# NIRVANALAN/CVPR23-E3DGE

Hardware: AMD Instinct MI355X
Metric: rendered_rays_per_sec_64x64x24 (higher is better)
Workload: dtype f32 (operands split f16 hi+lo, 3 f16 MFMA products, fp32 accumulate)

## Files before the change

cvpr23-e3dge_amd/_lib.py:

```python
import ctypes
import operator
import os
import threading
import weakref

_HERE = os.path.dirname(os.path.abspath(__file__))
LIB_PATH = os.environ.get("E3DGE_LIB_PATH") or os.path.join(_HERE, "lib", "libe3dge_hip.so")
ABI_VERSION = 17
PREC_F32, PREC_F16X3, PREC_F16X3_V1, PREC_F16X3_G2 = 0, 1, 2, 3
AMAX_FLOATS = 64 * 32
MC_MAX_TRIS = 16

_c_float_p = ctypes.c_void_p
_i32, _i64, _f32, _vp = ctypes.c_int, ctypes.c_int64, ctypes.c_float, ctypes.c_void_p


class _Args(ctypes.Structure):

    def __init__(self, *values, **fields):
        if values:
            fields = dict(zip((f[0] for f in self._fields_), values), **fields)
        seen = None
        for name, value in fields.items():
            kind = value.__class__
# ... 80 lines not shown
class Dec2Rgb(_Args):
    _fields_ = [(n, _vp) for n in ("weight", "style", "bias", "wm", "out")] + [("scale", _f32), ("ci", _i32)]


class Dec2Plan(_Args):
    _fields_ = [("batch", _i32), ("n_up", _i32), ("in_res", _i32), ("in_ch", _i32),
                ("features", _vp), ("skip_in", _vp), ("mod_table", _vp), ("latent", _vp),
                ("n_mod", _i32), ("mod_rows", _i32), ("mod_co", _i32), ("n_latent", _i32), ("style_dim", _i32), ("reserved0", _i32),
                ("conv1", Dec2Conv), ("rgb1", Dec2Rgb),
                ("up", Dec2Conv * DEC2_MAX_UP), ("conv", Dec2Conv * DEC2_MAX_UP), ("rgb", Dec2Rgb * DEC2_MAX_UP),
                ("act", _vp * (2 * DEC2_MAX_UP + 2)), ("amax", _vp), ("meta", _vp),
                ("fir_blur", _vp), ("fir_up", _vp), ("negative_slope", _f32), ("act_scale", _f32),
                ("kernel_ms", ctypes.POINTER(ctypes.c_float)), ("n_kernel_ms", _i32), ("reserved1", _i32),
                ("fir_blur_1d", _f32 * 4), ("fir_blur_separable", _i32), ("save_for_backward", _i32)]


class Dec2BwdConv(_Args):
    _fields_ = [(n, _vp) for n in ("wpre_t", "wcol", "wimg_t")]


class Dec2BwdPlan(_Args):
    _fields_ = [("d_img", _vp), ("d_features", _vp), ("conv1", Dec2BwdConv), ("up", Dec2BwdConv * DEC2_MAX_UP),
                ("conv", Dec2BwdConv * DEC2_MAX_UP), ("gact", _vp * (2 * DEC2_MAX_UP + 2)), ("pbuf", _vp),
                ("drgb", _vp * DEC2_MAX_UP), ("amax", _vp), ("meta", _vp), ("bounds", _vp),
                ("kernel_ms", ctypes.POINTER(ctypes.c_float)), ("n_kernel_ms", _i32), ("reserved", _i32),
                ("d_latent", _vp), ("ds_part", _vp), ("ds_part_floats", _i64)]


class WsLinear(_Args):
    _fields_ = [(n, _vp) for n in ("wimg", "x", "amax_in", "bias", "colw", "m", "r1", "r2", "y", "amax_out")] + [("n_rows", _i64)] + [
        (n, _i32) for n in ("ld_x", "off_x", "ld_m", "off_m", "ld_r1", "off_r1", "ld_r2", "off_r2", "ld_y", "off_y", "pre_relu", "post")] + [
        ("slope", _f32), ("w_fuse", _f32), ("xmul", _vp), ("amax_xmul", _vp), ("ld_xmul", _i32), ("off_xmul", _i32), ("x_scale", _f32),
        ("reserved", _i32)]


class Wgrad(_Args):
    _fields_ = [(n, _vp) for n in ("a", "amax_a", "b", "amax_b", "c", "ws")] + [("ws_floats", _i64), ("n_rows", _i64)] + [
        (n, _i32) for n in ("lda", "off_a", "m", "ldb", "off_b", "n", "ldc", "relu_b")] + [(n, _vp) for n in ("xcol", "colsum", "ccol")] + [
        (n, _i32) for n in ("ld_xcol", "ld_ccol", "b_gap_at", "b_gap")]


MESH_MAX_FACES_PER_PIXEL = 8


class MeshRenderArgs(_Args):
    _fields_ = [(n, _vp) for n in ("verts", "faces", "normals", "colors")] + [("n_verts", _i64), ("n_faces", _i64), ("camera", _f32 * 12),
               ("tan_half_fov", _f32), ("znear", _f32), ("zfar", _f32)] + [
        (n, _f32 * 3) for n in ("light_location", "ambient_color", "diffuse_color", "specular_color", "background_color")] + [
        ("blur_radius", _f32), ("sigma", _f32), ("gamma", _f32), ("image_size", _i32), ("faces_per_pixel", _i32)] + [
        (n, _vp) for n in ("image", "zbuf", "pix_to_face", "status", "ws")] + [("ws_bytes", _i64), ("bin_capacity", _i64)]


NOISE_PROJECT_FACES_PER_PIXEL, NOISE_PROJECT_MAX_MAPS = 17, 4


class NoiseProjectArgs(_Args):
    _fields_ = [(n, _vp) for n in ("verts", "faces", "vert_noise", "prev")] + [("n_verts", _i64), ("n_faces", _i64), ("camera", _f32 * 12)] + [
        (n, _f32) for n in ("tan_half_fov", "znear", "zfar", "blur_radius", "sigma", "gamma")] + [("image_size", _i32), ("n_maps", _i32)] + [
        (n, _vp) for n in ("out", "valid", "status", "ws")] + [("ws_bytes", _i64), ("bin_capacity", _i64)]


LPIPS_LAYERS = 5


class LpipsArgs(_Args):
    _fields_ = [(n, _vp) for n in ("packed", "x", "y")] + [(n, _i32) for n in ("batch", "height", "width", "reserved")] + [
# ... 197 lines not shown
    "e3dge_idnet_embed": (_i32, [ctypes.POINTER(IdnetArgs), _vp]),
    "e3dge_id_loss": (_i32, [ctypes.POINTER(IdLossArgs), _vp]),
    "e3dge_idnet_conv_tiles": (_i32, [_i32] * 5),
    "e3dge_idnet_conv": (_i32, [_vp] * 8 + [_i32] * 7 + [_vp]),
    "e3dge_idnet_packed_t_floats": (_i64, []),
    "e3dge_idnet_pack_weights_t": (_i32, [_vp, _vp, _vp]),
    "e3dge_idnet_saved_bytes": (_i64, [_i32]),
    "e3dge_idnet_embed_save": (_i32, [ctypes.POINTER(IdnetSaveArgs), _vp]),
    "e3dge_idnet_bwd_ws_bytes": (_i64, [_i32, _i32, _i32]),
    "e3dge_idnet_backward": (_i32, [ctypes.POINTER(IdnetBwdArgs), _vp]),
    "e3dge_idnet_conv_bwd": (_i32, [_vp] * 9 + [_i32] * 7 + [_vp]),
    "e3dge_idnet_prep_bwd": (_i32, [_vp, _vp, _i32, _i32, _i32, _vp]),
    "e3dge_hitprob_points": (_i32, [_vp] * 8 + [_i32, _i64, _i32, _i32, _vp]),
    "e3dge_hitprob_composite": (_i32, [_vp] * 6 + [_f32, _i32, _i32, _i64, _i32, _i32, _vp]),
    "e3dge_align_volume": (_i32, [_vp, _vp, _vp, _vp, _vp, _vp, _i32, _i32, _i32, _i32, _i32, _vp]),
    "e3dge_marching_cubes_ws_bytes": (_i64, [_i32, _i32, _i32]),
    "e3dge_marching_cubes_count": (_i32, [_vp, _vp, _i64, _vp, _i32, _i32, _i32, _i64, _i64, _i64, _vp]),
    "e3dge_marching_cubes_emit": (_i32, [_vp, _vp, _i64, _i64, _vp, _i64, _vp, _i32, _i32, _i32, _i64, _i64, _i64, _i32, _vp]),
    "e3dge_marching_cubes_tables": (_i32, [_vp, _vp]),
    "e3dge_depth_mesh": (_i32, [_vp, _vp, _vp, _i32, _i32, _vp]),
    "e3dge_vertex_normals_ws_bytes": (_i64, [_i64]),
    "e3dge_vertex_normals": (_i32, [_vp, _vp, _vp, _i64, _i64, _vp, _i64, _vp]),
    "e3dge_mesh_render_ws_bytes": (_i64, [_i64, _i64, _i32, _i64]),
    "e3dge_mesh_render": (_i32, [ctypes.POINTER(MeshRenderArgs), _vp]),
    "e3dge_mesh_subdivide": (_i32, [_vp, _vp, _vp, _vp, _vp, _vp, _i64, _i64, _i64, _vp]),
    "e3dge_noise_project_ws_bytes": (_i64, [_i64, _i64, _i32, _i64]),
    "e3dge_noise_project": (_i32, [ctypes.POINTER(NoiseProjectArgs), _vp]),
    "e3dge_selftest_mfma": (_i32, [_vp, _vp, _vp, _i32, _vp]),
    "e3dge_selftest_mfma16": (_i32, [_vp, _vp, _vp, _i32, _vp]),
    "e3dge_selftest_mfma16x16": (_i32, [_vp, _vp, _vp, _i32, _vp]),
    "e3dge_ws_image_bytes": (_i64, [_i32]),
    "e3dge_ws_pack": (_i32, [_vp, _vp, _i32, _vp]),
    "e3dge_ws_linear": (_i32, [ctypes.POINTER(WsLinear), _vp]),
    "e3dge_ws_rowdot2": (_i32, [_vp, _i32, _i32, _vp, _vp, _vp, _vp, _vp, _i32, _i32, _i64, _vp]),
    "e3dge_selftest_sin": (_i32, [_vp, _vp, _i32, _vp]),
    "e3dge_selftest_sin_poly": (_i32, [_vp, _vp, _i32, _vp]),
    "e3dge_avgpool_fwd": (_i32, [_vp, _vp, _i64, _i32, _i32, _i32, _vp]),
    "e3dge_avgpool_bwd": (_i32, [_vp, _vp, _i64, _i32, _i32, _i32, _vp]),
    "e3dge_sqerr_bwd": (_i32, [_vp, _vp, _vp, _i64, _vp, _vp]),
    "e3dge_shape_loss_partial_floats": (_i64, [ctypes.POINTER(ShapeLossArgs)]),
    "e3dge_shape_loss_fwd": (_i32, [ctypes.POINTER(ShapeLossArgs), _vp]),
    "e3dge_shape_loss_bwd": (_i32, [ctypes.POINTER(ShapeLossArgs), _vp]),
    "e3dge_disc_packed_floats": (_i64, [_i32] * 3),
    "e3dge_disc_pack_weights": (_i32, [_vp, _vp, _vp]),
    "e3dge_disc_ws_bytes": (_i64, [_i32] * 7),
    "e3dge_disc_saved_bytes": (_i64, [_i32] * 4),
    "e3dge_disc_forward": (_i32, [ctypes.POINTER(DiscArgs), _vp]),
    "e3dge_disc_backward": (_i32, [ctypes.POINTER(DiscBwdArgs), _vp]),
    "e3dge_disc_conv": (_i32, [_vp] * 6 + [_i32] * 9 + [_f32, _vp]),
    "e3dge_disc_conv_dgrad": (_i32, [_vp] * 5 + [_f32, _f32, _vp] + [_i32] * 7 + [_f32, _vp]),
    "e3dge_disc_stddev": (_i32, [_vp, _vp, _vp, _i32, _i32, _i32, _vp]),
    "e3dge_hgf_packed_floats": (_i64, [_i32, _i32]),
    "e3dge_hgf_pack_weights": (_i32, [_vp, _vp, _i32, _vp, _i32, _i32, _vp]),
    "e3dge_hgf_ws_bytes": (_i64, [_i32] * 5),
    "e3dge_hgf_forward": (_i32, [ctypes.POINTER(HgfArgs), _vp]),
    "e3dge_hgf_front": (_i32, [_vp] * 4 + [_i32] * 5 + [_vp, _i64, _vp]),
    "e3dge_hgf_conv": (_i32, [_vp] * 8 + [_i32] * 12 + [_vp]),
    "e3dge_hgf_norm": (_i32, [_vp] * 4 + [_i32] * 7 + [_vp]),
    "e3dge_hgf_pool": (_i32, [_vp, _vp, _i64, _i32, _i32, _vp]),
    "e3dge_hgf_up_add": (_i32, [_vp, _vp, _vp, _i64, _i32, _i32, _vp]),
    "e3dge_hgf_saved_bytes": (_i64, [_i32] * 5),
    "e3dge_hgf_forward_saving": (_i32, [ctypes.POINTER(HgfArgs), _vp, _i64, _vp]),
    "e3dge_hgf_front_saving": (_i32, [_vp] * 4 + [_i32] * 5 + [_vp, _i64, _vp, _i64, _vp]),
    "e3dge_hgf_packed_t_floats": (_i64, [_i32, _i32]),
    "e3dge_hgf_pack_weights_t": (_i32, [_vp, _vp, _i32, _vp, _i32, _i32, _vp]),
    "e3dge_hgf_bwd_ws_bytes": (_i64, [_i32] * 5),
# ... 266 lines not shown
```

cvpr23-e3dge_amd/build.py:

```python
import hashlib
import os
import shutil
import subprocess
import sys

HERE = os.path.dirname(os.path.abspath(__file__))
CSRC = os.path.join(HERE, "csrc")
LIBDIR = os.path.join(HERE, "lib")
LIBNAME = "libe3dge_hip.so"
SOURCES = ["stream_ops.hip", "upfirdn2d.hip", "siren.hip", "siren_bwd.hip", "resblock.hip", "modconv.hip", "decoder2.hip", "local_query.hip", "metrics.hip", "align_volume.hip", "hitprob.hip", "siren_ws.hip", "wgrad.hip",
           "marching_cubes.hip", "mesh_render.hip", "lpips.hip", "idnet.hip", "losses.hip", "disc.hip", "hgfilter.hip", "aligner.hip"]
ARCH = "gfx950"
FLAGS = ["-O3", "-std=c++17", "-fPIC", f"--offload-arch={ARCH}", "-ffp-contract=on", "-fno-slp-vectorize",
         "-Wno-unused-result"]


def lib_path():
    return os.path.join(LIBDIR, LIBNAME)


def _hipcc():
    for cand in (os.environ.get("HIPCC"), shutil.which("hipcc"), "/opt/rocm/bin/hipcc"):
        if cand and os.path.exists(cand):
            return cand
    raise RuntimeError("hipcc not found (set HIPCC=...)")


def _digest():
    h = hashlib.sha256()
    for name in sorted(os.listdir(CSRC)) + ["../../include/e3dge_hip.h"]:
        with open(os.path.join(CSRC, name), "rb") as f:
            h.update(name.encode() + b"\0" + f.read())
    h.update(" ".join(FLAGS).encode())
    return h.hexdigest()


def _compile(pairs, flags, verbose, jobs):
    hipcc = _hipcc()
    todo, running = list(pairs), []
    while todo or running:
        while todo and len(running) < jobs:
            src, obj = todo.pop(0)
            cmd = [hipcc, *flags, "-c", os.path.join(CSRC, src), "-o", obj]
# ... 63 lines not shown
```

cvpr23-e3dge_amd/local_query.py:

```python
import os

import torch
from torch import nn

from . import _lib


def fuse_autograd_backend():
    v = os.environ.get("E3DGE_FUSE_AUTOGRAD", "hip")
    if v not in ("hip", "torch"):
        raise RuntimeError(f"E3DGE_FUSE_AUTOGRAD must be 'hip' or 'torch', got {v!r}")
    return v


def native_fuse_backend():
    v = os.environ.get("E3DGE_FUSE", "hip")
    if v not in ("hip", "torch"):
        raise RuntimeError(f"E3DGE_FUSE must be 'hip' or 'torch', got {v!r}")
    return v


def query_feature_map(pts, calibs, fmap=None, out=None, col_off=0, mask_out=None, mask_off=0, want_proj=False):
    _lib.require_gpu(pts, "pts")
    _lib.require_gpu(calibs, "calibs")
# ... 178 lines not shown
        if fc0.out_features != 256 or self.encode_enc.fc_1.out_features != 256 or fc0.in_features not in (512, 513):
            return False
        if enc_in.shape[-1] != fc0.in_features or self.encode_enc.shortcut is None:
            return False
        return all(p.device == enc_in.device and p.dtype == torch.float32 for p in _lib.params_of(self))

    def _fusefn_ok(self, enc_in, dec_feat, w):
        if enc_in.numel() == 0 or (torch.is_tensor(w) and (w.requires_grad or w.numel() != 1)):
            return False
        b_off = enc_in.shape[-1] - 256
        tail = enc_in[..., b_off:]
        return (torch.is_tensor(dec_feat) and dec_feat.shape == tail.shape and dec_feat.data_ptr() == tail.data_ptr()
                and dec_feat.stride() == tail.stride())

    def _wants_grad(self, enc_in):
        return torch.is_grad_enabled() and (enc_in.requires_grad or any(p.requires_grad for p in _lib.params_of(self)))

    def _param_list(self):
        e = self.encode_enc
        return [e.fc_0.weight, e.fc_0.bias, e.fc_1.weight, e.fc_1.bias, e.shortcut.weight,
                self.scale[0].weight, self.scale[0].bias, self.scale[2].weight, self.scale[2].bias,
                self.shift[0].weight, self.shift[0].bias, self.shift[2].weight, self.shift[2].bias]

    def invalidate(self):
        _lib.invalidate(self)

    def _images(self, device):
        return _lib.cached(self, 'images', _lib.params_of(self), self._build_images, (str(device),))

    def _build_images(self):
        enc, n_in = self.encode_enc, self.encode_enc.fc_0.in_features
        has_col = n_in == 513
        b_off = 257 if has_col else 256
        img = _ws_image
        f0, sc = enc.fc_0.weight, enc.shortcut.weight
        return dict(b_off=b_off, has_col=has_col,
                    f0a=img(f0[:, :256]), f0b=img(f0[:, b_off:]), f1=img(enc.fc_1.weight), sa=img(sc[:, :256]), sb=img(sc[:, b_off:]),
                    sc1=img(self.scale[0].weight), sc2=img(self.scale[2].weight), sh1=img(self.shift[0].weight), sh2=img(self.shift[2].weight),
                    f0col=f0[:, 256].detach().contiguous() if has_col else None, scol=sc[:, 256].detach().contiguous() if has_col else None,
                    b0=enc.fc_0.bias.detach().contiguous(), b1=enc.fc_1.bias.detach().contiguous(),
                    bsc1=self.scale[0].bias.detach().contiguous(), bsc2=self.scale[2].bias.detach().contiguous(),
                    bsh1=self.shift[0].bias.detach().contiguous(), bsh2=self.shift[2].bias.detach().contiguous(),
                    slope=float(self.scale[1].negative_slope))

    def _images_t(self, device):
        I = self._images(device)
        if 'sc2_t' not in I:
            enc, b_off = self.encode_enc, I['b_off']
            img_t = lambda w: _ws_image(w.t())
            f0, sc = enc.fc_0.weight, enc.shortcut.weight
            I.update(sc2_t=img_t(self.scale[2].weight), sh2_t=img_t(self.shift[2].weight), sc1_t=img_t(self.scale[0].weight),
                     sh1_t=img_t(self.shift[0].weight), f1_t=img_t(enc.fc_1.weight), sa_t=img_t(sc[:, :256]), sb_t=img_t(sc[:, b_off:]),
                     f0a_t=img_t(f0[:, :256]), f0b_t=img_t(f0[:, b_off:]))
        return I

    def _fuse_bwd_native(self, g, x, net, s1, t1, scale, am_x, w, b_off, slope, need_x, ld_g=256, mask_col=True):
        N = g.shape[0]
        dev = g.device
        ld = x.shape[1]
        I = self._images_t(dev)
        f32 = dict(device=dev, dtype=torch.float32)
        dz1, dz2, de, dnet = (torch.empty((N, 256), **f32) for _ in range(4))
        dx = torch.empty((N, ld), **f32) if need_x else None
        am = torch.zeros((5, _lib.AMAX_FLOATS), **f32)

        def lin(wimg, xin, am_in, y, ld_x=256, ld_y=256, off_y=0, post=0, sl=0.0, r1=None, r1_ld=256, r1_off=0, r2=None, r2_ld=256, r2_off=0,
                xmul=None, amax_out=None, x_scale=1.0):
            a = _lib.WsLinear()
            a.wimg, a.x, a.amax_in, a.y, a.amax_out = wimg, xin, am_in, y, amax_out
            a.r1, a.r2 = r1, r2
            a.n_rows = N
            a.ld_x, a.off_x, a.ld_y, a.off_y = ld_x, 0, ld_y, off_y
            a.ld_r1, a.off_r1, a.ld_r2, a.off_r2, a.ld_m, a.off_m = r1_ld, r1_off, r2_ld, r2_off, 1, 0
            a.post, a.slope, a.w_fuse, a.x_scale = post, sl, w, x_scale
            if xmul is not None:
                a.xmul, a.amax_xmul, a.ld_xmul, a.off_xmul = xmul, am_x, ld, b_off
# ... 2 lines not shown
            _lib.launch("e3dge_amax", am[0], g, g.numel())
        else:
            _lib.launch("e3dge_amax_rows", am[0], g, N, 256, ld_g)
        lin(I['sc2_t'], g, am[0], dz1, ld_x=ld_g, post=3, sl=slope, r1=s1, xmul=x, x_scale=w, amax_out=am[1])
        lin(I['sh2_t'], g, am[0], dz2, ld_x=ld_g, post=3, sl=slope, r1=t1, x_scale=w, amax_out=am[2])
        lin(I['sc1_t'], dz1, am[1], de)
        lin(I['sh1_t'], dz2, am[2], de, r1=de, amax_out=am[3])
        lin(I['f1_t'], de, am[3], dnet, post=3, sl=0.0, r1=net, amax_out=am[4])
        if need_x:
            lin(I['sa_t'], de, am[3], dx, ld_y=ld, off_y=0)
            lin(I['f0a_t'], dnet, am[4], dx, ld_y=ld, off_y=0, post=3, sl=0.0, r1=x, r1_ld=ld, r1_off=0, r2=dx, r2_ld=ld, r2_off=0)
            lin(I['sb_t'], de, am[3], dx, ld_y=ld, off_y=b_off, post=4, r1=g, r1_ld=ld_g, r2=scale)
            lin(I['f0b_t'], dnet, am[4], dx, ld_y=ld, off_y=b_off, post=3, sl=0.0, r1=x, r1_ld=ld, r1_off=b_off, r2=dx, r2_ld=ld, r2_off=b_off)
        if need_x and I['has_col'] and not mask_col:
            dx[:, 256].zero_()
        if need_x and I['has_col'] and mask_col:
            _lib.launch("e3dge_ws_rowdot2", dx, ld, 256, de, I['scol'], dnet, I['f0col'], x, ld, 256, N)
        return dz1, dz2, de, dnet, dx, am

    def _fuse_native(self, enc_in, w, out, out_off, keep=None):
        lead = enc_in.shape[:-1]
        x = _lib.dense(enc_in.reshape(-1, enc_in.shape[-1]))
        N, ld = x.shape
        dev = x.device
        I = self._images(dev)
        if out is None:
            out = torch.empty(lead + (256,), device=dev, dtype=torch.float32)
            out_off = 0
        o2 = out.reshape(-1, out.shape[-1])
        if o2.data_ptr() != out.data_ptr() or not o2.is_contiguous():
            raise RuntimeError("Fuse_sft_MLP.fuse: `out` must be a contiguous (..., ld) buffer")
        if N == 0:
            return out[..., out_off:out_off + 256]
        A, Bf, C = (torch.empty((N, 256), device=dev, dtype=torch.float32) for _ in range(3))
        if keep is not None:
            NET, E, S1, T1 = (torch.empty((N, 256), device=dev, dtype=torch.float32) for _ in range(4))
        else:
            NET, E, S1, T1 = Bf, Bf, A, A
        am = torch.zeros((5, _lib.AMAX_FLOATS), device=dev, dtype=torch.float32)
        b_off = I['b_off']

        def lin(wimg, xin, ld_x, off_x, amax_in, y, ld_y=256, off_y=0, bias=None, col=None, r1=None, r1_ld=256, r1_off=0, r2=None,
                pre_relu=False, post=0, amax_out=None):
            a = _lib.WsLinear()
            a.wimg, a.x, a.amax_in, a.bias = wimg, xin, amax_in, bias
            a.colw, a.m = (col, x) if col is not None else (None, None)
            a.r1, a.r2, a.y, a.amax_out = r1, r2, y, amax_out
            a.n_rows = N
            a.ld_x, a.off_x, a.ld_m, a.off_m = ld_x, off_x, ld, 256
            a.ld_r1, a.off_r1, a.ld_r2, a.off_r2, a.ld_y, a.off_y = r1_ld, r1_off, 256, 0, ld_y, off_y
            a.pre_relu, a.post, a.slope, a.w_fuse = int(pre_relu), post, I['slope'], w
            _lib.launch("e3dge_ws_linear", a)
        _lib.launch("e3dge_amax", am[0], x, x.numel())
        lin(I['f0a'], x, ld, 0, am[0], A, pre_relu=True)
        lin(I['f0b'], x, ld, b_off, am[0], NET, bias=I['b0'], col=I['f0col'], r1=A, pre_relu=True, amax_out=am[1])
        lin(I['f1'], NET, 256, 0, am[1], A, bias=I['b1'], pre_relu=True)
        lin(I['sa'], x, ld, 0, am[0], C)
        lin(I['sb'], x, ld, b_off, am[0], E, col=I['scol'], r1=C, r2=A, amax_out=am[2])
        lin(I['sc1'], E, 256, 0, am[2], S1, bias=I['bsc1'], post=1, amax_out=am[3])
        lin(I['sc2'], S1, 256, 0, am[3], C, bias=I['bsc2'])
        lin(I['sh1'], E, 256, 0, am[2], T1, bias=I['bsh1'], post=1, amax_out=am[4])
        lin(I['sh2'], T1, 256, 0, am[4], o2, ld_y=o2.shape[-1], off_y=out_off, bias=I['bsh2'], r1=x, r1_ld=ld, r1_off=b_off, r2=C, post=2)
        if keep is not None:
            keep.update(x=x, net=NET, e=E, s1=S1, t1=T1, scale=C, b_off=b_off, slope=I['slope'], am_x=am[0], am=am)
        return out[..., out_off:out_off + 256]


class _FuseFn(torch.autograd.Function):

    @staticmethod
    def forward(ctx, mod, enc_in, w, pe_pts, n_freqs, mask_col_const, *params):
        keep = {}
        with torch.no_grad():
            if pe_pts is None:
                out = mod._fuse_native(enc_in.detach(), w, None, 0, keep=keep)
            else:
                width = 3 * (2 * n_freqs + 1)
                out = torch.empty(enc_in.shape[:-1] + (256 + width,), device=enc_in.device, dtype=torch.float32)
                mod._fuse_native(enc_in.detach(), w, out, 0, keep=keep)
                pos_encoding(pe_pts.detach(), n_freqs, out=out.reshape(-1, 256 + width), col_off=256)
        ctx.mod, ctx.w, ctx.in_shape, ctx.mask_col_const = mod, w, enc_in.shape, bool(mask_col_const)
        ctx.b_off, ctx.slope, ctx.am_x, ctx.am_fwd = keep['b_off'], keep['slope'], keep['am_x'], keep['am']
        ctx.save_for_backward(keep['x'], keep['net'], keep['e'], keep['s1'], keep['t1'], keep['scale'], *params)
        return out

    @staticmethod
    @torch.autograd.function.once_differentiable
    def backward(ctx, grad_out):
        x, net, e, s1, t1, scale = ctx.saved_tensors[:6]
        W0, _, W1, _, Ws, Wsc1, _, Wsc2, _, Wsh1, _, Wsh2, _ = ctx.saved_tensors[6:]
        w, b_off, slope = ctx.w, ctx.b_off, ctx.slope
        need = ctx.needs_input_grad[6:]
        need_x = ctx.needs_input_grad[1]
        g_rows = grad_out.reshape(-1, grad_out.shape[-1]).float()
        rows_ok = g_rows.stride(-1) == 1 and (g_rows.shape[0] <= 1 or g_rows.stride(0) >= g_rows.shape[1]) and g_rows.data_ptr() % 16 == 0
# ... 129 lines not shown
```

include/e3dge_hip.h:

```cpp
#ifndef E3DGE_HIP_H
#define E3DGE_HIP_H

#include <stdint.h>

#ifdef __cplusplus
extern "C" {
#endif

typedef void* e3dge_stream_t;

enum {
    E3DGE_OK = 0,
    E3DGE_ERR_INVALID_ARG = -1,
    E3DGE_ERR_LAUNCH = -2,
    E3DGE_ERR_UNSUPPORTED = -3
};

int e3dge_abi_version(void);
int e3dge_build_flags(void);
int64_t e3dge_stream_capture_id(e3dge_stream_t stream);
const char* e3dge_last_error(void);


int e3dge_fused_bias_act(float* y, const float* x, const float* bias, const float* ref, int act,
// ... 437 lines not shown
    int64_t n_verts, n_faces;
    float camera[12];
    float tan_half_fov, znear, zfar;
    float blur_radius, sigma, gamma;
    int32_t image_size, n_maps;
    float* out; uint8_t* valid;
    int32_t* status;
    void* ws;
    int64_t ws_bytes, bin_capacity;
} E3dgeNoiseProjectArgs;
int e3dge_mesh_subdivide(float* out_verts, int32_t* out_faces, const float* verts, const int32_t* faces, const int64_t* edge_keys,
                         const int32_t* side_rank, int64_t n_verts, int64_t n_faces, int64_t n_edges, e3dge_stream_t stream);
int64_t e3dge_noise_project_ws_bytes(int64_t n_verts, int64_t n_faces, int image_size, int64_t bin_capacity);
int e3dge_noise_project(const E3dgeNoiseProjectArgs* args, e3dge_stream_t stream);

int e3dge_selftest_mfma(float* c, const float* a, const float* b, int k, e3dge_stream_t stream);
int e3dge_selftest_mfma16(float* c, const float* a, const float* b, int k, e3dge_stream_t stream);
int e3dge_selftest_mfma16x16(float* c, const float* a, const float* b, int k, e3dge_stream_t stream);
int64_t e3dge_ws_image_bytes(int n_layers);
int e3dge_ws_pack(void* wimg, const float* weights, int n_layers, e3dge_stream_t stream);
typedef struct E3dgeWsLinear {
    const void* wimg; const float* x; const float* amax_in; const float* bias; const float* colw; const float* m;
    const float* r1; const float* r2; float* y; float* amax_out;
    int64_t n_rows;
    int32_t ld_x, off_x, ld_m, off_m, ld_r1, off_r1, ld_r2, off_r2, ld_y, off_y;
    int32_t pre_relu, post;
    float slope, w_fuse;
    const float* xmul; const float* amax_xmul;
    int32_t ld_xmul, off_xmul;
    float x_scale;
    int32_t reserved;
} E3dgeWsLinear;
int e3dge_ws_linear(const E3dgeWsLinear* args, e3dge_stream_t stream);
int e3dge_ws_rowdot2(float* out, int ld_out, int off_out, const float* a, const float* u, const float* b, const float* v, const float* gate,
                     int ld_gate, int off_gate, int64_t n_rows, e3dge_stream_t stream);
typedef struct E3dgeWgrad {
    const float* a; const float* amax_a; const float* b; const float* amax_b;
    float* c; float* ws;
    int64_t ws_floats, n_rows;
    int32_t lda, off_a, m, ldb, off_b, n, ldc, relu_b;
    const float* xcol; float* colsum; float* ccol;
    int32_t ld_xcol, ld_ccol, b_gap_at, b_gap;
} E3dgeWgrad;
int64_t e3dge_wgrad_ws_floats(int m, int n, int64_t n_rows);
int e3dge_wgrad(const E3dgeWgrad* args, e3dge_stream_t stream);
int e3dge_selftest_sin(float* y, const float* x, int n, e3dge_stream_t stream);
int e3dge_selftest_sin_poly(float* y, const float* x, int n, e3dge_stream_t stream);

int e3dge_avgpool_fwd(float* out, const float* in, int64_t planes, int in_h, int in_w, int f, e3dge_stream_t stream);
int e3dge_avgpool_bwd(float* d_in, const float* d_out, int64_t planes, int in_h, int in_w, int f, e3dge_stream_t stream);
int e3dge_sqerr_bwd(float* d_pred, const float* pred, const float* gt, int64_t n, const float* scale_ptr, e3dge_stream_t stream);
#define E3DGE_SHAPE_LOSS_SEGMENTS 4
#define E3DGE_SHAPE_SMOOTH_L1 0
#define E3DGE_SHAPE_EIKONAL 1
typedef struct E3dgeShapeLossSegment {
    const float* pred; const float* gt; float* d_pred;
    int64_t n;
    float lambda;
    int32_t kind;
} E3dgeShapeLossSegment;
typedef struct E3dgeShapeLossArgs {
    E3dgeShapeLossSegment seg[E3DGE_SHAPE_LOSS_SEGMENTS];
    float* terms; float* total; float* partial;
    int64_t partial_floats;
    const float* upstream;
} E3dgeShapeLossArgs;
// ... 234 lines not shown
```

Baseline: 14.42 million.

## Fuse Fuse_sft_MLP linear chain into one persistent MFMA kernel

Replaces eight separate weight-stationary linear launches plus an amax pass with a single persistent kernel. The kernel keeps each 64-row tile's intermediates in LDS as split f16 hi/lo, applies per-row power-of-two scaling, and streams the packed weights through a register ring. Only the last shift linear stays a separate launch. Intermediates are no longer written to and reread from global memory, and launch overhead drops, at the cost of heavy LDS/register use, low occupancy, and a new per-row scaling scheme whose numerics differ from the old global-amax scaling.

```diff
diff --git a/cvpr23-e3dge_amd/_lib.py b/cvpr23-e3dge_amd/_lib.py
--- a/cvpr23-e3dge_amd/_lib.py
+++ b/cvpr23-e3dge_amd/_lib.py
@@ -136,6 +136,11 @@
         (n, _i32) for n in ("ld_x", "off_x", "ld_m", "off_m", "ld_r1", "off_r1", "ld_r2", "off_r2", "ld_y", "off_y", "pre_relu", "post")] + [
         ("slope", _f32), ("w_fuse", _f32), ("xmul", _vp), ("amax_xmul", _vp), ("ld_xmul", _i32), ("off_xmul", _i32), ("x_scale", _f32),
         ("reserved", _i32)]
+
+
+class FuseChain(_Args):
+    _fields_ = [(n, _vp) for n in ("wimg", "x", "scale", "t1", "net", "e", "s1", "amax")] + [("n_rows", _i64), ("ld_x", _i32), ("b_off", _i32),
+                                                                                          ("slope", _f32), ("save", _i32)]
 
 
 class Wgrad(_Args):
@@ -399,6 +404,9 @@
     "e3dge_ws_image_bytes": (_i64, [_i32]),
     "e3dge_ws_pack": (_i32, [_vp, _vp, _i32, _vp]),
     "e3dge_ws_linear": (_i32, [ctypes.POINTER(WsLinear), _vp]),
+    "e3dge_fuse_chain_image_bytes": (_i64, []),
+    "e3dge_fuse_chain_pack": (_i32, [_vp] * 12 + [_i32, _vp]),
+    "e3dge_fuse_chain_fwd": (_i32, [ctypes.POINTER(FuseChain), _vp]),
     "e3dge_ws_rowdot2": (_i32, [_vp, _i32, _i32, _vp, _vp, _vp, _vp, _vp, _i32, _i32, _i64, _vp]),
     "e3dge_selftest_sin": (_i32, [_vp, _vp, _i32, _vp]),
     "e3dge_selftest_sin_poly": (_i32, [_vp, _vp, _i32, _vp]),
diff --git a/cvpr23-e3dge_amd/build.py b/cvpr23-e3dge_amd/build.py
--- a/cvpr23-e3dge_amd/build.py
+++ b/cvpr23-e3dge_amd/build.py
@@ -8,7 +8,7 @@
 CSRC = os.path.join(HERE, "csrc")
 LIBDIR = os.path.join(HERE, "lib")
 LIBNAME = "libe3dge_hip.so"
-SOURCES = ["stream_ops.hip", "upfirdn2d.hip", "siren.hip", "siren_bwd.hip", "resblock.hip", "modconv.hip", "decoder2.hip", "local_query.hip", "metrics.hip", "align_volume.hip", "hitprob.hip", "siren_ws.hip", "wgrad.hip",
+SOURCES = ["stream_ops.hip", "upfirdn2d.hip", "siren.hip", "siren_bwd.hip", "resblock.hip", "modconv.hip", "decoder2.hip", "local_query.hip", "metrics.hip", "align_volume.hip", "hitprob.hip", "siren_ws.hip", "fuse_chain.hip", "wgrad.hip",
            "marching_cubes.hip", "mesh_render.hip", "lpips.hip", "idnet.hip", "losses.hip", "disc.hip", "hgfilter.hip", "aligner.hip"]
 ARCH = "gfx950"
 FLAGS = ["-O3", "-std=c++17", "-fPIC", f"--offload-arch={ARCH}", "-ffp-contract=on", "-fno-slp-vectorize",
diff --git a/cvpr23-e3dge_amd/csrc/fuse_chain.hip b/cvpr23-e3dge_amd/csrc/fuse_chain.hip
--- /dev/null
+++ b/cvpr23-e3dge_amd/csrc/fuse_chain.hip
@@ -0,0 +1,462 @@
+#define E3DGE_16_HELPERS_ONLY
+#include <string.h>
+#include "siren16.h"
+
+namespace e3dge {
+
+constexpr int kFcThreads = 512;
+constexpr int kFcRows = 64;
+constexpr int kFcUnits = 64;
+constexpr int kFcUnitVec = 4 * 64;
+constexpr int kFcRing = 4;
+constexpr int kFcHalfBytes = 8 * 4 * 1024;
+constexpr int kFcBufBytes = 2 * kFcHalfBytes;
+constexpr int kFcVecs = 7;
+constexpr int64_t kFcImgWeightBytes = (int64_t)8 * kFcUnits * kFcUnitVec * 16;
+constexpr int64_t kFcImgBytes = kFcImgWeightBytes + kFcVecs * kWidth * 4;
+constexpr int kFcLdsBytes = 2 * kFcBufBytes + kFcVecs * kWidth * 4 + kFcRows * 8 * 4;
+static_assert(kFcLdsBytes <= 160 * 1024, "LDS budget");
+static_assert(kFcUnits % kFcRing == 0, "the ring slot of a unit is the same in every tile");
+constexpr float kFcLoUp = 1024.0f, kFcLoDown = 1.0f / 1024.0f;
+constexpr int kFcU_W1 = 32, kFcU_Sft = 40, kFcU_Sc2 = 56;
+
+struct FuseChainK {
+    const u32x4* wimg; const float* x; float* scale; float* t1; float* net; float* e; float* s1; float* amax;
+    int64_t n_rows;
+    int ld_x, b_off;
+    float slope;
+    int save;
+};
+
+struct __attribute__((packed, aligned(4))) FcF4U { float v[4]; };
+typedef short fc_s16x2 __attribute__((ext_vector_type(2)));
+
+__device__ __forceinline__ void fc_relu_hilo(unsigned& h, unsigned& l) {
+    const fc_s16x2 hv = __builtin_bit_cast(fc_s16x2, h);
+    const unsigned neg = __builtin_bit_cast(unsigned, hv >> (fc_s16x2){15, 15});
+    h = __builtin_bit_cast(unsigned, __builtin_elementwise_max(hv, (fc_s16x2){0, 0}));
+    l &= ~neg;
+}
+__device__ __forceinline__ u32x4 fc_times(u32x4 v, float pow2) {
+    const _Float16 r = (_Float16)pow2;
+    const half8 r8 = {r, r, r, r, r, r, r, r};
+    return __builtin_bit_cast(u32x4, __builtin_bit_cast(half8, v) * r8);
+}
+__device__ __forceinline__ float fc_max_over_q(float m) {
+    m = fmaxf(m, __shfl_xor(m, 16, kWave));
+    return fmaxf(m, __shfl_xor(m, 32, kWave));
+}
+__device__ __forceinline__ void fc_row_scale(float m, float& sc, float& inv) {
+    const unsigned e = min(max((__float_as_uint(m) >> 23) & 255u, 24u), 254u);
+    sc = __uint_as_float((267u - e) << 23);
+    inv = __uint_as_float((e - 20u) << 23);
+}
+
+struct FcAcc { f32x4v t[2][4]; };
+struct FcB { u32x4 h[4], s[4], l[4]; };
+
+template <bool SAVE>
+__global__ void __launch_bounds__(kFcThreads) fuse_chain_kernel(const FuseChainK a) {
+    extern __shared__ __attribute__((aligned(16))) char smem[];
+    char* const bufP = smem;
+    char* const bufQ = smem + kFcBufBytes;
+    float* const vec = reinterpret_cast<float*>(smem + 2 * kFcBufBytes);
+    float* const tab = vec + kFcVecs * kWidth;
+    const int tid = threadIdx.x, lane = tid & 63, wave = __builtin_amdgcn_readfirstlane(tid >> 6), n = lane & 15, q = lane >> 4;
+    const int64_t n_tiles = (a.n_rows + kFcRows - 1) / kFcRows, last_row = a.n_rows - 1;
+    const bool has_col = a.b_off == kWidth + 1;
+    {
+        const float* vsrc = reinterpret_cast<const float*>(reinterpret_cast<const char*>(a.wimg) + kFcImgWeightBytes);
+        for (int i = tid; i < kFcVecs * kWidth; i += kFcThreads) vec[i] = vsrc[i];
+    }
+    const float* const b0_s = vec, *const b1_s = vec + kWidth, *const bsc1_s = vec + 2 * kWidth, *const bsh1_s = vec + 3 * kWidth,
+                *const bsc2_s = vec + 4 * kWidth, *const f0col_s = vec + 5 * kWidth, *const scol_s = vec + 6 * kWidth;
+
+    const char* __restrict__ const wbase = reinterpret_cast<const char*>(a.wimg + (size_t)wave * kFcUnits * kFcUnitVec);
+    const unsigned wvoff = (unsigned)lane * 16u;
+    u32x4 W[kFcRing][4];
+    auto load_unit = [&](int u) {
+        const int uu = u % kFcUnits;
+        unsigned uoff = uu * (kFcUnitVec * 16);
+        asm volatile("" : "+s"(uoff));
+#pragma unroll
+        for (int j = 0; j < 4; ++j) W[uu % kFcRing][j] = *reinterpret_cast<const u32x4*>(wbase + uoff + (wvoff + j * 1024));
+    };
+#pragma unroll
+    for (int u = 0; u < kFcRing - 1; ++u) load_unit(u);
+
+    auto load_b = [&](FcB& b, const char* buf, int g) {
+        const char* p = buf + g * 4096 + lane * 16;
+#pragma unroll
+        for (int pt = 0; pt < 4; ++pt) {
+            b.h[pt] = *reinterpret_cast<const u32x4*>(p + pt * 1024);
+            b.l[pt] = *reinterpret_cast<const u32x4*>(p + pt * 1024 + kFcHalfBytes);
+        }
+    };
+    auto down_b = [&](FcB& b) {
+#pragma unroll
+        for (int pt = 0; pt < 4; ++pt) b.s[pt] = fc_times(b.h[pt], kFcLoDown);
+    };
+    auto relu_b = [&](FcB& b) {
+#pragma unroll
+        for (int pt = 0; pt < 4; ++pt)
+#pragma unroll
+            for (int w = 0; w < 4; ++w) { unsigned h = b.h[pt][w], l = b.l[pt][w]; fc_relu_hilo(h, l); b.h[pt][w] = h; b.l[pt][w] = l; }
+    };
+    auto mma_unit = [&](int u, const FcB& b, FcAcc& acc) {
+        load_unit(u + kFcRing - 1);
+        const u32x4 (&w)[4] = W[u % kFcRing];
+#pragma unroll
+        for (int pass = 0; pass < 3; ++pass)
+#pragma unroll
+            for (int ft = 0; ft < 2; ++ft)
+#pragma unroll
+                for (int pt = 0; pt < 4; ++pt)
+                    acc.t[ft][pt] = mfma16x16(pass == 1 ? w[2 * ft + 1] : w[2 * ft], pass == 0 ? b.h[pt] : pass == 1 ? b.s[pt] : b.l[pt], acc.t[ft][pt]);
+        __builtin_amdgcn_sched_barrier(0);
+    };
+    auto zero_acc = [](FcAcc& acc) {
+#pragma unroll
+        for (int ft = 0; ft < 2; ++ft)
+#pragma unroll
+            for (int pt = 0; pt < 4; ++pt) acc.t[ft][pt] = zero4();
+    };
+
+    f32x4 xa0[4], xa1[4], xb0[4], xb1[4];
+    float mcol[4];
+    auto stage_load = [&](int64_t tile, int parts) {
+        int lane_o = lane;
+        asm volatile("" : "+v"(lane_o));
+        const int n = lane_o & 15, q = lane_o >> 4;
+#pragma unroll
+        for (int t = 0; t < 4; ++t) {
+            const int64_t row = tile * kFcRows + 16 * t + n;
+            const float* p = a.x + (row <= last_row ? row : last_row) * a.ld_x;
+            if (parts & 1) {
+                const FcF4U u0 = *reinterpret_cast<const FcF4U*>(p + 32 * wave + 8 * q), u1 = *reinterpret_cast<const FcF4U*>(p + 32 * wave + 8 * q + 4);
+                const float mc = p[kWidth];
+#pragma unroll
+                for (int i = 0; i < 4; ++i) { xa0[t][i] = u0.v[i]; xa1[t][i] = u1.v[i]; }
+                mcol[t] = mc;
+            }
+            if (parts & 2) {
+                const FcF4U v0 = *reinterpret_cast<const FcF4U*>(p + a.b_off + 32 * wave + 8 * q), v1 = *reinterpret_cast<const FcF4U*>(p + a.b_off + 32 * wave + 8 * q + 4);
+#pragma unroll
+                for (int i = 0; i < 4; ++i) { xb0[t][i] = v0.v[i]; xb1[t][i] = v1.v[i]; }
+            }
+        }
+    };
+    auto put8 = [&](char* o, const f32x4& u, const f32x4& w, float sc) {
+        const HiLo p0 = split2(u[0] * sc, u[1] * sc), p1 = split2(u[2] * sc, u[3] * sc), p2 = split2(w[0] * sc, w[1] * sc), p3 = split2(w[2] * sc, w[3] * sc);
+        *reinterpret_cast<u32x4*>(o) = u32x4{p0.h, p1.h, p2.h, p3.h};
+        *reinterpret_cast<u32x4*>(o + kFcHalfBytes) = u32x4{p0.l, p1.l, p2.l, p3.l};
+    };
+    auto row_scales = [&](const float (&bm)[4], float (&sc)[4], float (&inv)[4]) {
+        int lane_o = lane;
+        asm volatile("" : "+v"(lane_o));
+#pragma unroll
+        for (int pt = 0; pt < 4; ++pt) {
+            const float m = fc_max_over_q(bm[pt]);
+            if ((lane_o >> 4) == 0) tab[(16 * pt + (lane_o & 15)) * 8 + wave] = m;
+        }
+        __syncthreads();
+#pragma unroll
+        for (int pt = 0; pt < 4; ++pt) {
+            const f32x4v i0 = *reinterpret_cast<const f32x4v*>(tab + (16 * pt + (lane_o & 15)) * 8), i1 = *reinterpret_cast<const f32x4v*>(tab + (16 * pt + (lane_o & 15)) * 8 + 4);
+            const float m = fmaxf(fmaxf(fmaxf(i0[0], i0[1]), fmaxf(i0[2], i0[3])), fmaxf(fmaxf(i1[0], i1[1]), fmaxf(i1[2], i1[3])));
+            fc_row_scale(m, sc[pt], inv[pt]);
+        }
+    };
+    auto put_acc = [&](char* buf, const FcAcc& v, const float (&sc)[4]) {
+        int lane_o = lane;
+        asm volatile("" : "+v"(lane_o));
+        const int n = lane_o & 15, q = lane_o >> 4;
+#pragma unroll
+        for (int pt = 0; pt < 4; ++pt)
+#pragma unroll
+            for (int ft = 0; ft < 2; ++ft) {
+                const HiLo p0 = split2(v.t[ft][pt][0] * sc[pt], v.t[ft][pt][1] * sc[pt]), p1 = split2(v.t[ft][pt][2] * sc[pt], v.t[ft][pt][3] * sc[pt]);
+                char* o = buf + ((wave * 4 + pt) * 4 + 2 * ft + (q >> 1)) * 256 + n * 16 + 8 * (q & 1);
+                *reinterpret_cast<uint2*>(o) = uint2{p0.h, p1.h};
+                *reinterpret_cast<uint2*>(o + kFcHalfBytes) = uint2{p0.l, p1.l};
+            }
+    };
+
+    float am_net = 0.0f, am_e = 0.0f, am_s1 = 0.0f, am_t1 = 0.0f;
+    stage_load(blockIdx.x, 3);
+    for (int64_t tile = blockIdx.x; tile < n_tiles; tile += gridDim.x) {
+        float inv_x[4], mraw[4];
+        {
+            float bm[4], sc[4];
+#pragma unroll
+            for (int t = 0; t < 4; ++t) {
+                float m = 0.0f;
+#pragma unroll
+                for (int i = 0; i < 4; ++i) m = fmaxf(m, fmaxf(fmaxf(fabsf(xa0[t][i]), fabsf(xa1[t][i])), fmaxf(fabsf(xb0[t][i]), fabsf(xb1[t][i]))));
+                bm[t] = m;
+                mraw[t] = has_col ? mcol[t] : 0.0f;
+            }
+            row_scales(bm, sc, inv_x);
+#pragma unroll
+            for (int t = 0; t < 4; ++t) {
+                char* o = ((wave * 4 + t) * 4 + q) * 256 + n * 16 + bufP;
+                put8(o, xa0[t], xa1[t], sc[t]);
+                put8(o + kFcBufBytes, xb0[t], xb1[t], sc[t]);
+            }
+            __syncthreads();
+        }
+        bool ok[4];
+#pragma unroll
+        for (int pt = 0; pt < 4; ++pt) ok[pt] = tile * kFcRows + 16 * pt + n <= last_row;
+        const int64_t tile_off = tile * (kFcRows * kWidth);
+        auto first_feature = [&]() { int l = lane; asm volatile("" : "+v"(l)); return 32 * wave + 4 * (l >> 4); };
+        auto store4 = [&](float* out, int f0, int pt, int ft, const f32x4v& v) {
+            int l = lane;
+            asm volatile("" : "+v"(l));
+            *reinterpret_cast<f32x4v*>((out + tile_off + (pt * 16 * kWidth + 16 * ft)) + (unsigned)((l & 15) * kWidth + f0)) = v;
+        };
+
+        FcAcc S, N;
+        zero_acc(S); zero_acc(N);
+#pragma unroll
+        for (int g = 0; g < 16; ++g) {
+            FcB b;
+            load_b(b, g < 8 ? bufP : bufQ, g & 7);
+            down_b(b);
+            mma_unit(2 * g, b, S);
+            relu_b(b);
+            down_b(b);
+            mma_unit(2 * g + 1, b, N);
+        }
+        float inv_n[4];
+        {
+            float bm[4], sc[4];
+            const int f0 = first_feature();
+#pragma unroll
+            for (int pt = 0; pt < 4; ++pt) {
+                const float mv = fmaxf(mraw[pt], 0.0f);
+                float m = 0.0f;
+#pragma unroll
+                for (int ft = 0; ft < 2; ++ft) {
+                    const f32x4v b4 = *reinterpret_cast<const f32x4v*>(b0_s + f0 + 16 * ft), c4 = *reinterpret_cast<const f32x4v*>(f0col_s + f0 + 16 * ft);
+                    f32x4v v;
+#pragma unroll
+                    for (int i = 0; i < 4; ++i) {
+                        v[i] = fmaf(c4[i], mv, fmaf(N.t[ft][pt][i], inv_x[pt], b4[i]));
+                        if (SAVE && ok[pt]) am_net = fmaxf(am_net, fabsf(v[i]));
+                        N.t[ft][pt][i] = fmaxf(v[i], 0.0f);
+                        m = fmaxf(m, N.t[ft][pt][i]);
+                    }
+                    if (SAVE && ok[pt]) store4(a.net, f0, pt, ft, v);
+                }
+                bm[pt] = m;
+            }
+            row_scales(bm, sc, inv_n);
+            put_acc(bufP, N, sc);
+            __syncthreads();
+        }
+        float inv_e[4];
+        {
+            zero_acc(N);
+#pragma unroll
+            for (int g = 0; g < 8; ++g) {
+                FcB b;
+                load_b(b, bufP, g);
+                down_b(b);
+                mma_unit(kFcU_W1 + g, b, N);
+            }
+            float bm[4], sc[4];
+            const int f0 = first_feature();
+#pragma unroll
+            for (int pt = 0; pt < 4; ++pt) {
+                float m = 0.0f;
+#pragma unroll
+                for (int ft = 0; ft < 2; ++ft) {
+                    const f32x4v b4 = *reinterpret_cast<const f32x4v*>(b1_s + f0 + 16 * ft), c4 = *reinterpret_cast<const f32x4v*>(scol_s + f0 + 16 * ft);
+                    f32x4v v;
+#pragma unroll
+                    for (int i = 0; i < 4; ++i) {
+                        v[i] = fmaf(c4[i], mraw[pt], fmaf(S.t[ft][pt][i], inv_x[pt], fmaf(N.t[ft][pt][i], inv_n[pt], b4[i])));
+                        m = fmaxf(m, fabsf(v[i]));
+                        S.t[ft][pt][i] = v[i];
+                    }
+                    if (SAVE && ok[pt]) store4(a.e, f0, pt, ft, v);
+                }
+                if (SAVE && ok[pt]) am_e = fmaxf(am_e, m);
+                bm[pt] = m;
+            }
+            row_scales(bm, sc, inv_e);
+            put_acc(bufQ, S, sc);
+            __syncthreads();
+        }
+        float inv_s[4];
+        {
+            zero_acc(S); zero_acc(N);
+#pragma unroll
+            for (int g = 0; g < 8; ++g) {
+                FcB b;
+                load_b(b, bufQ, g);
+                down_b(b);
+                mma_unit(kFcU_Sft + 2 * g, b, S);
+                mma_unit(kFcU_Sft + 2 * g + 1, b, N);
+            }
+            float bm[4], sc[4];
+            const int f0 = first_feature();
+#pragma unroll
+            for (int pt = 0; pt < 4; ++pt) {
+                float m = 0.0f, mt = 0.0f;
+#pragma unroll
+                for (int ft = 0; ft < 2; ++ft) {
+                    const f32x4v b4 = *reinterpret_cast<const f32x4v*>(bsc1_s + f0 + 16 * ft), d4 = *reinterpret_cast<const f32x4v*>(bsh1_s + f0 + 16 * ft);
+                    f32x4v v, u;
+#pragma unroll
+                    for (int i = 0; i < 4; ++i) {
+                        const float s = fmaf(S.t[ft][pt][i], inv_e[pt], b4[i]), t = fmaf(N.t[ft][pt][i], inv_e[pt], d4[i]);
+                        v[i] = fmaxf(s, s * a.slope);
+                        u[i] = fmaxf(t, t * a.slope);
+                        m = fmaxf(m, fabsf(v[i]));
+                        mt = fmaxf(mt, fabsf(u[i]));
+                        S.t[ft][pt][i] = v[i];
+                    }
+                    if (ok[pt]) store4(a.t1, f0, pt, ft, u);
+                    if (SAVE && ok[pt]) store4(a.s1, f0, pt, ft, v);
+                }
+                if (SAVE && ok[pt]) { am_s1 = fmaxf(am_s1, m); am_t1 = fmaxf(am_t1, mt); }
+                bm[pt] = m;
+            }
+            row_scales(bm, sc, inv_s);
+            put_acc(bufP, S, sc);
+            __syncthreads();
+        }
+        {
+            const int64_t nxt = tile + gridDim.x, nxt_c = nxt < n_tiles ? nxt : n_tiles - 1;
+            stage_load(nxt_c, SAVE ? 1 : 3);
+            zero_acc(N);
+#pragma unroll
+            for (int g = 0; g < 8; ++g) {
+                FcB b;
+                load_b(b, bufP, g);
+                down_b(b);
+                mma_unit(kFcU_Sc2 + g, b, N);
+            }
+            if (SAVE) stage_load(nxt_c, 2);
+            const int f0 = first_feature();
+#pragma unroll
+            for (int pt = 0; pt < 4; ++pt)
+#pragma unroll
+                for (int ft = 0; ft < 2; ++ft) {
+                    const f32x4v b4 = *reinterpret_cast<const f32x4v*>(bsc2_s + f0 + 16 * ft);
+                    f32x4v v;
+#pragma unroll
+                    for (int i = 0; i < 4; ++i) v[i] = fmaf(N.t[ft][pt][i], inv_s[pt], b4[i]);
+                    if (ok[pt]) store4(a.scale, f0, pt, ft, v);
+                }
+        }
+    }
+    if (SAVE) {
+        const float am[4] = {am_net, am_e, am_s1, am_t1};
+#pragma unroll
+        for (int r = 0; r < 4; ++r) {
+            const float m = wave_max(am[r]);
+            if (lane == 0) atomic_max_nonneg(a.amax + (r + 1) * (kAmaxSlots * kAmaxStride) + (((int)blockIdx.x * 8 + wave) & (kAmaxSlots - 1)) * kAmaxStride, m);
+        }
+    }
+    asm volatile("s_waitcnt vmcnt(0)" ::: "memory");
+}
+
+struct FuseChainPackK {
+    const float* w0; const float* ws; const float* w1; const float* wsc1; const float* wsh1; const float* wsc2;
+    const float* b0; const float* b1; const float* bsc1; const float* bsh1; const float* bsc2;
+    int n_in;
+};
+__global__ void __launch_bounds__(256) fuse_chain_pack_kernel(unsigned* __restrict__ img, const FuseChainPackK a) {
+    const int64_t n_words = kFcImgWeightBytes / 4, n_all = kFcImgBytes / 4;
+    const int b_off = a.n_in - kWidth;
+    for (int64_t e = (int64_t)blockIdx.x * 256 + threadIdx.x; e < n_all; e += (int64_t)gridDim.x * 256) {
+        if (e >= n_words) {
+            const int i = (int)(e - n_words), which = i >> 8, f = i & 255;
+            float v;
+            switch (which) {
+                case 0: v = a.b0[f]; break;
+                case 1: v = a.b1[f]; break;
+                case 2: v = a.bsc1[f]; break;
+                case 3: v = a.bsh1[f]; break;
+                case 4: v = a.bsc2[f]; break;
+                case 5: v = b_off == kWidth + 1 ? a.w0[(int64_t)f * a.n_in + kWidth] : 0.0f; break;
+                default: v = b_off == kWidth + 1 ? a.ws[(int64_t)f * a.n_in + kWidth] : 0.0f; break;
+            }
+            img[e] = __float_as_uint(v);
+            continue;
+        }
+        int64_t r = e;
+        const int wd = r & 3; r >>= 2;
+        const int lane = r & 63; r >>= 6;
+        const int hl = r & 1; r >>= 1;
+        const int ft = r & 1; r >>= 1;
+        const int unit = r & 63; r >>= 6;
+        const int wave = (int)r;
+        const float* w;
+        int ld = kWidth, col0 = 0, g;
+        if (unit < kFcU_W1) {
+            g = unit >> 1;
+            w = (unit & 1) ? a.w0 : a.ws;
+            ld = a.n_in;
+            col0 = g >= 8 ? b_off : 0;
+            g &= 7;
+        } else if (unit < kFcU_Sft) {
+            g = unit - kFcU_W1; w = a.w1;
+        } else if (unit < kFcU_Sc2) {
+            g = (unit - kFcU_Sft) >> 1; w = ((unit - kFcU_Sft) & 1) ? a.wsh1 : a.wsc1;
+        } else {
+            g = unit - kFcU_Sc2; w = a.wsc2;
+        }
+        const int f = 32 * wave + 16 * ft + (lane & 15), k = col0 + 32 * g + 8 * (lane >> 4) + 2 * wd;
+        const float* src = w + (int64_t)f * ld + k;
+        const float s0 = src[0] * kW16Scale, s1 = src[1] * kW16Scale;
+        const unsigned h = __builtin_bit_cast(unsigned, __builtin_amdgcn_cvt_pkrtz(s0, s1));
+        const unsigned l = __builtin_bit_cast(unsigned, __builtin_amdgcn_cvt_pkrtz((s0 - f16lo(h)) * kFcLoUp, (s1 - f16hi(h)) * kFcLoUp));
+        img[e] = hl ? l : h;
+    }
+}
+
+}
+
+using namespace e3dge;
+
+extern "C" int64_t e3dge_fuse_chain_image_bytes(void) { return kFcImgBytes; }
+
+extern "C" int e3dge_fuse_chain_pack(void* wimg, const float* w0, const float* ws, const float* w1, const float* wsc1, const float* wsh1,
+                                     const float* wsc2, const float* b0, const float* b1, const float* bsc1, const float* bsh1,
+                                     const float* bsc2, int n_in, e3dge_stream_t stream) {
+    E3DGE_REQUIRE(wimg && w0 && ws && w1 && wsc1 && wsh1 && wsc2 && b0 && b1 && bsc1 && bsh1 && bsc2, "fuse_chain_pack: null pointer");
+    E3DGE_REQUIRE(n_in == 2 * kWidth || n_in == 2 * kWidth + 1, "fuse_chain_pack: n_in=%d, must be 512 or 513", n_in);
+    E3DGE_REQUIRE((reinterpret_cast<uintptr_t>(wimg) & 15) == 0, "fuse_chain_pack: the image must be 16-byte aligned");
+    const FuseChainPackK k{w0, ws, w1, wsc1, wsh1, wsc2, b0, b1, bsc1, bsh1, bsc2, n_in};
+    fuse_chain_pack_kernel<<<dim3(1024), dim3(256), 0, as_stream(stream)>>>(reinterpret_cast<unsigned*>(wimg), k);
+    return check_launch("fuse_chain_pack");
+}
+
+static_assert(sizeof(E3dgeFuseChain) == sizeof(e3dge::FuseChainK), "E3dgeFuseChain mirrors FuseChainK");
+
+extern "C" int e3dge_fuse_chain_fwd(const E3dgeFuseChain* args, e3dge_stream_t stream) {
+    E3DGE_REQUIRE(args && args->wimg && args->x && args->scale && args->t1, "fuse_chain_fwd: null pointer");
+    E3DGE_REQUIRE(!args->save || (args->net && args->e && args->s1 && args->amax), "fuse_chain_fwd: the saving form needs net, e, s1 and amax");
+    E3DGE_REQUIRE(args->n_rows >= 0, "fuse_chain_fwd: n_rows=%lld", (long long)args->n_rows);
+    E3DGE_REQUIRE(args->b_off == kWidth || args->b_off == kWidth + 1, "fuse_chain_fwd: b_off=%d, must be 256 or 257", args->b_off);
+    E3DGE_REQUIRE(args->ld_x >= args->b_off + kWidth, "fuse_chain_fwd: two 256-column blocks must fit the row pitch (ld_x %d, b_off %d)", args->ld_x, args->b_off);
+    E3DGE_REQUIRE(args->slope >= 0.0f && args->slope <= 1.0f, "fuse_chain_fwd: leaky slope must be in [0, 1]");
+    uintptr_t al = reinterpret_cast<uintptr_t>(args->wimg) | reinterpret_cast<uintptr_t>(args->scale) | reinterpret_cast<uintptr_t>(args->t1);
+    if (args->save) al |= reinterpret_cast<uintptr_t>(args->net) | reinterpret_cast<uintptr_t>(args->e) | reinterpret_cast<uintptr_t>(args->s1);
+    E3DGE_REQUIRE((al & 15) == 0 && (reinterpret_cast<uintptr_t>(args->x) & 3) == 0, "fuse_chain_fwd: wimg and the (n_rows, 256) outputs must be 16-byte aligned");
+    if (args->n_rows == 0) return E3DGE_OK;
+    FuseChainK k;
+    memcpy(&k, args, sizeof(k));
+    const void* fn = k.save ? reinterpret_cast<const void*>(&fuse_chain_kernel<true>) : reinterpret_cast<const void*>(&fuse_chain_kernel<false>);
+    hipError_t e = hipFuncSetAttribute(fn, hipFuncAttributeMaxDynamicSharedMemorySize, kFcLdsBytes);
+    if (e != hipSuccess) return fail(E3DGE_ERR_LAUNCH, "hipFuncSetAttribute(fuse_chain): %s", hipGetErrorString(e));
+    const int64_t n_tiles = (k.n_rows + kFcRows - 1) / kFcRows;
+    const unsigned grid = (unsigned)(n_tiles < 256 ? n_tiles : 256);
+    if (k.save) fuse_chain_kernel<true><<<dim3(grid), dim3(kFcThreads), kFcLdsBytes, as_stream(stream)>>>(k);
+    else fuse_chain_kernel<false><<<dim3(grid), dim3(kFcThreads), kFcLdsBytes, as_stream(stream)>>>(k);
+    return check_launch("fuse_chain_fwd");
+}
diff --git a/cvpr23-e3dge_amd/local_query.py b/cvpr23-e3dge_amd/local_query.py
--- a/cvpr23-e3dge_amd/local_query.py
+++ b/cvpr23-e3dge_amd/local_query.py
@@ -234,16 +234,15 @@
         enc, n_in = self.encode_enc, self.encode_enc.fc_0.in_features
         has_col = n_in == 513
         b_off = 257 if has_col else 256
-        img = _ws_image
         f0, sc = enc.fc_0.weight, enc.shortcut.weight
-        return dict(b_off=b_off, has_col=has_col,
-                    f0a=img(f0[:, :256]), f0b=img(f0[:, b_off:]), f1=img(enc.fc_1.weight), sa=img(sc[:, :256]), sb=img(sc[:, b_off:]),
-                    sc1=img(self.scale[0].weight), sc2=img(self.scale[2].weight), sh1=img(self.shift[0].weight), sh2=img(self.shift[2].weight),
-                    f0col=f0[:, 256].detach().contiguous() if has_col else None, scol=sc[:, 256].detach().contiguous() if has_col else None,
-                    b0=enc.fc_0.bias.detach().contiguous(), b1=enc.fc_1.bias.detach().contiguous(),
-                    bsc1=self.scale[0].bias.detach().contiguous(), bsc2=self.scale[2].bias.detach().contiguous(),
-                    bsh1=self.shift[0].bias.detach().contiguous(), bsh2=self.shift[2].bias.detach().contiguous(),
-                    slope=float(self.scale[1].negative_slope))
+        d = lambda p: p.detach().contiguous()
+        chain = torch.empty(_lib.query("e3dge_fuse_chain_image_bytes"), dtype=torch.uint8, device=f0.device)
+        _lib.launch("e3dge_fuse_chain_pack", chain, d(f0), d(sc), d(enc.fc_1.weight), d(self.scale[0].weight), d(self.shift[0].weight),
+                    d(self.scale[2].weight), d(enc.fc_0.bias), d(enc.fc_1.bias), d(self.scale[0].bias), d(self.shift[0].bias),
+                    d(self.scale[2].bias), n_in)
+        return dict(b_off=b_off, has_col=has_col, chain=chain, sh2=_ws_image(self.shift[2].weight),
+                    f0col=d(f0[:, 256]) if has_col else None, scol=d(sc[:, 256]) if has_col else None,
+                    bsh2=d(self.shift[2].bias), slope=float(self.scale[1].negative_slope))
 
     def _images_t(self, device):
         I = self._images(device)
@@ -312,35 +311,25 @@
             raise RuntimeError("Fuse_sft_MLP.fuse: `out` must be a contiguous (..., ld) buffer")
         if N == 0:
             return out[..., out_off:out_off + 256]
-        A, Bf, C = (torch.empty((N, 256), device=dev, dtype=torch.float32) for _ in range(3))
+        f32 = dict(device=dev, dtype=torch.float32)
+        C, T1 = torch.empty((N, 256), **f32), torch.empty((N, 256), **f32)
+        b_off = I['b_off']
+        c = _lib.FuseChain()
+        c.wimg, c.x, c.scale, c.t1 = I['chain'], x, C, T1
+        c.n_rows, c.ld_x, c.b_off, c.slope, c.save = N, ld, b_off, I['slope'], int(keep is not None)
         if keep is not None:
-            NET, E, S1, T1 = (torch.empty((N, 256), device=dev, dtype=torch.float32) for _ in range(4))
-        else:
-            NET, E, S1, T1 = Bf, Bf, A, A
-        am = torch.zeros((5, _lib.AMAX_FLOATS), device=dev, dtype=torch.float32)
-        b_off = I['b_off']
-
-        def lin(wimg, xin, ld_x, off_x, amax_in, y, ld_y=256, off_y=0, bias=None, col=None, r1=None, r1_ld=256, r1_off=0, r2=None,
-                pre_relu=False, post=0, amax_out=None):
-            a = _lib.WsLinear()
-            a.wimg, a.x, a.amax_in, a.bias = wimg, xin, amax_in, bias
-            a.colw, a.m = (col, x) if col is not None else (None, None)
-            a.r1, a.r2, a.y, a.amax_out = r1, r2, y, amax_out
-            a.n_rows = N
-            a.ld_x, a.off_x, a.ld_m, a.off_m = ld_x, off_x, ld, 256
-            a.ld_r1, a.off_r1, a.ld_r2, a.off_r2, a.ld_y, a.off_y = r1_ld, r1_off, 256, 0, ld_y, off_y
-            a.pre_relu, a.post, a.slope, a.w_fuse = int(pre_relu), post, I['slope'], w
-            _lib.launch("e3dge_ws_linear", a)
-        _lib.launch("e3dge_amax", am[0], x, x.numel())
-        lin(I['f0a'], x, ld, 0, am[0], A, pre_relu=True)
-        lin(I['f0b'], x, ld, b_off, am[0], NET, bias=I['b0'], col=I['f0col'], r1=A, pre_relu=True, amax_out=am[1])
-        lin(I['f1'], NET, 256, 0, am[1], A, bias=I['b1'], pre_relu=True)
-        lin(I['sa'], x, ld, 0, am[0], C)
-        lin(I['sb'], x, ld, b_off, am[0], E, col=I['scol'], r1=C, r2=A, amax_out=am[2])
-        lin(I['sc1'], E, 256, 0, am[2], S1, bias=I['bsc1'], post=1, amax_out=am[3])
-        lin(I['sc2'], S1, 256, 0, am[3], C, bias=I['bsc2'])
-        lin(I['sh1'], E, 256, 0, am[2], T1, bias=I['bsh1'], post=1, amax_out=am[4])
-        lin(I['sh2'], T1, 256, 0, am[4], o2, ld_y=o2.shape[-1], off_y=out_off, bias=I['bsh2'], r1=x, r1_ld=ld, r1_off=b_off, r2=C, post=2)
+            NET, E, S1 = (torch.empty((N, 256), **f32) for _ in range(3))
+            am = torch.zeros((5, _lib.AMAX_FLOATS), **f32)
+            _lib.launch("e3dge_amax", am[0], x, x.numel())
+            c.net, c.e, c.s1, c.amax = NET, E, S1, am
+        _lib.launch("e3dge_fuse_chain_fwd", c)
+        a = _lib.WsLinear()
+        a.wimg, a.x, a.bias, a.r1, a.r2, a.y = I['sh2'], T1, I['bsh2'], x, C, o2
+        a.n_rows = N
+        a.ld_x, a.off_x, a.ld_m, a.off_m = 256, 0, ld, 256
+        a.ld_r1, a.off_r1, a.ld_r2, a.off_r2, a.ld_y, a.off_y = ld, b_off, 256, 0, o2.shape[-1], out_off
+        a.pre_relu, a.post, a.slope, a.w_fuse = 0, 2, I['slope'], w
+        _lib.launch("e3dge_ws_linear", a)
         if keep is not None:
             keep.update(x=x, net=NET, e=E, s1=S1, t1=T1, scale=C, b_off=b_off, slope=I['slope'], am_x=am[0], am=am)
         return out[..., out_off:out_off + 256]
diff --git a/include/e3dge_hip.h b/include/e3dge_hip.h
--- a/include/e3dge_hip.h
+++ b/include/e3dge_hip.h
@@ -493,6 +493,17 @@
     int32_t reserved;
 } E3dgeWsLinear;
 int e3dge_ws_linear(const E3dgeWsLinear* args, e3dge_stream_t stream);
+typedef struct E3dgeFuseChain {
+    const void* wimg; const float* x; float* scale; float* t1; float* net; float* e; float* s1; float* amax;
+    int64_t n_rows;
+    int32_t ld_x, b_off;
+    float slope;
+    int32_t save;
+} E3dgeFuseChain;
+int64_t e3dge_fuse_chain_image_bytes(void);
+int e3dge_fuse_chain_pack(void* wimg, const float* w0, const float* ws, const float* w1, const float* wsc1, const float* wsh1, const float* wsc2,
+                          const float* b0, const float* b1, const float* bsc1, const float* bsh1, const float* bsc2, int n_in, e3dge_stream_t stream);
+int e3dge_fuse_chain_fwd(const E3dgeFuseChain* args, e3dge_stream_t stream);
 int e3dge_ws_rowdot2(float* out, int ld_out, int off_out, const float* a, const float* u, const float* b, const float* v, const float* gate,
                      int ld_gate, int off_gate, int64_t n_rows, e3dge_stream_t stream);
 typedef struct E3dgeWgrad {
```

Result: no change. 14.38 million (-0.2%).
